# jasonyaw/CDAE

Measured on AMD Instinct MI355X. Metric: users/sec (whole node) K=200 ML-10M-shape; Recall@10 parity, higher is better.
Workload: dtype f32

## Files before the change

### cdae_amd/csrc/cdae_hip.hip

```cpp
#include <hip/hip_runtime.h>

#include <cstring>

#include <rocprim/rocprim.hpp>

#include <algorithm>
#include <atomic>
#include <condition_variable>
#include <deque>
#include <mutex>
#include <thread>
#include <chrono>
#include <cmath>
#include <cstdarg>
#include <cstdlib>
#include <cstdio>
#include <cstring>
#include <numeric>
#include <string>
#include <vector>

#include "../../include/cdae_hip.h"
#include "cdae_internal.hpp"
#include "cdae_kernels.hpp"
// ... 163 lines not shown
  double* d_rows_out = nullptr;
  int sort_bits = 1;
  struct PrepJob { int set; uint64_t s0; uint32_t nb, cidx; uint64_t E; uint64_t seed; uint32_t epoch; int lane; uint64_t prof_q; };
  bool prep_threaded = true;
  std::thread worker;
  std::mutex job_mu;
  std::condition_variable job_cv;
  std::condition_variable issued_cv;
  std::deque<PrepJob> jobs;
  bool worker_stop = false;
  uint64_t jobs_submitted = 0;
  std::atomic<uint64_t> jobs_issued{0};
  std::atomic<int> worker_failed{0};
  std::string worker_error;
  std::mutex prof_mu;
  bool encode_two_launches = false;
  bool debug_skip_prep = false;
  bool bucket_sort = false;
  uint32_t bucket_ranges = 0;
  uint32_t* d_bucket_cut = nullptr;
  bool bucket_attr_set = false;
  uint16_t* d_range_of = nullptr;
  uint32_t cell_units = 0;
  bool counting_sort = false;
  bool tile_attr_set = false;
  bool gemm3_attr_set[8] = {false, false, false, false, false, false, false, false};
  bool gemmw_attr_set[8] = {false, false, false, false, false, false, false, false};
  bool gemm_narrow = false;
  bool gemm1_tiled = false;
  bool gemm1_duo_attr_set[2] = {false, false};
  bool fused_attr_set = false;
  bool gemm2_nt = false;
  bool gemm_tn_attr_set = false;
  bool rows_separate = false;
  bool fused_rows_attr_set[2][2] = {};
  int rows_fused_kh = 2;

  float* d_base = nullptr; float* d_delta = nullptr; float* d_recv = nullptr; float* d_snap = nullptr;
  void* xchg = nullptr; void (*xchg_free)(void*) = nullptr;
  uint32_t delta_combine = CDAE_COMBINE_SUM;
  uint32_t mf = 0, mf_bias = 1;
  bool mf_seq = false;
  bool mf_auto = false;
  bool prep_force_sort = false;
  std::vector<uint32_t> user_perm, user_inv;
  uint32_t ex_per_pos = 1;
// ... 243 lines not shown
    hipLaunchKernelGGL(mf_sample_kernel, dim3((n_units + 3) / 4), dim3(256), 0, st, h->hp, h->mf == 2 ? 1u : 0u, h->d_row_ptr, h->d_col,
                       h->d_unit_ptr + bt.s0, n_units, bt.s0, bt.nb, seed, epoch, x.item, x.val, x.key16, x.seg, bucket ? 0u : 2u * I, x.dup_count,
                       x.dup_of_ex, h->d_unit_user, x.wg_state);
  } else if (shs) {
    hipLaunchKernelGGL(sample_kernel, dim3((n_units + 3) / 4), dim3(256), 0, st, h->hp, h->d_grow_ptr, h->d_gcol,
                       h->d_gunit_ptr + bt.s0, n_units, bt.s0, bt.nb, bt.cidx, seed, epoch, x.item, x.val, x.key16,
                       x.seg, h->counting_sort || bucket ? 0u : 4u * I, x.dup_count, x.dup_of_ex, h->d_gunit_user,
                       x.wg_state, (const uint32_t*)nullptr, (uint32_t)h->item0, I, (uint32_t)h->I_global,
                       (const uint16_t*)(use_cells ? h->d_range_of : nullptr), (const uint32_t*)h->d_bucket_cut, h->bucket_ranges,
                       use_cells ? x.cells : (uint32_t*)nullptr, x.cell_flag, x.cell_tag);
  } else
  hipLaunchKernelGGL(sample_kernel, dim3((n_units + 3) / 4), dim3(256), 0, st, h->hp, h->d_row_ptr, h->d_col,
                     h->d_unit_ptr + bt.s0, n_units, bt.s0, bt.nb, bt.cidx, seed, epoch, x.item, x.val, x.key16,
                     x.seg, h->counting_sort || bucket ? 0u : 4u * I, x.dup_count, x.dup_of_ex, h->d_unit_user,
                     x.wg_state, (const uint32_t*)h->d_gpos, 0u, 0u, 0u,
                     (const uint16_t*)(use_cells ? h->d_range_of : nullptr), (const uint32_t*)h->d_bucket_cut, h->bucket_ranges,
                     use_cells ? x.cells : (uint32_t*)nullptr, x.cell_flag, x.cell_tag);
  CHK(pr.end());
  CHK(pr.begin(h, F_SORT, st, prof_q));
  const dim3 seg_grid((uint32_t)((bt.E + 256 * SEG_PER_THREAD - 1) / (256 * SEG_PER_THREAD)));
  if (bt.E == 0) {
  } else if (h->mf_seq && !h->prep_force_sort) {
  } else if (bucket) {
    if (!h->bucket_attr_set) {
      HIPCHK(hipFuncSetAttribute((const void*)bucket_sort_kernel, hipFuncAttributeMaxDynamicSharedMemorySize, (int)BK_LDS_BYTES));
      h->bucket_attr_set = true;
    }
    hipLaunchKernelGGL(bucket_sort_kernel, dim3(h->bucket_ranges), dim3(BK_THREADS), BK_LDS_BYTES, st, (const uint16_t*)x.key16, (const uint64_t*)x.val,
                       (uint32_t)bt.E, (const uint32_t*)h->d_bucket_cut, x.wg_state, (const uint32_t*)(use_cells ? x.cells : nullptr), n_units,
                       (const uint32_t*)x.cell_flag, x.cell_tag, x.seg, x.seg + I, (const uint32_t*)h->d_rank_of,
                       x.seg + 2 * (size_t)I, x.seg + 3 * (size_t)I, x.sorted_val, x.bucketed, x.dup_count, h->dup_cap, x.dup_of_pos, x.dup_of_ex,
                       h->dup_stripes, h->d_fused_err);
  } else if (h->counting_sort) {
    const uint32_t n_tiles = (uint32_t)((bt.E + TILE_EX - 1) / TILE_EX);
    const size_t tile_lds = (size_t)I * sizeof(uint32_t);
    if (tile_lds + 1024 > 64 * 1024 && !h->tile_attr_set) {
      HIPCHK(hipFuncSetAttribute((const void*)tile_hist_kernel, hipFuncAttributeMaxDynamicSharedMemorySize, (int)tile_lds));
      HIPCHK(hipFuncSetAttribute((const void*)tile_scatter_kernel, hipFuncAttributeMaxDynamicSharedMemorySize, (int)tile_lds + 1024));
      h->tile_attr_set = true;
    }
    hipLaunchKernelGGL(tile_hist_kernel, dim3(n_tiles), dim3(TILE_THREADS), tile_lds / 2 + 4, st, x.item, (uint32_t)bt.E, I, x.tile_hist);
    hipLaunchKernelGGL(item_tile_scan_kernel, dim3((I + 255) / 256), dim3(256), 0, st, x.tile_hist, n_tiles, I, x.item_count, x.rank, x.block_total);
    hipLaunchKernelGGL(tile_scatter_kernel, dim3(n_tiles), dim3(TILE_THREADS), tile_lds + 128 * sizeof(uint32_t), st, x.item, x.val,
                       (uint32_t)bt.E, I, x.tile_hist, x.item_count, x.rank, x.block_total, x.prefix, x.seg, x.seg + I, x.dup_count, x.bucketed,
                       (const uint32_t*)h->d_rank_of, x.seg + 2 * (size_t)I, x.seg + 3 * (size_t)I);
    hipLaunchKernelGGL(segment_sort_kernel, dim3((I + SEGSORT_ITEMS - 1) / SEGSORT_ITEMS), dim3(SEGSORT_THREADS), 0, st, I, x.prefix, x.bucketed,
                       x.sorted_val, x.item_count, x.dup_count, h->dup_cap, x.dup_of_pos, x.dup_of_ex, h->dup_stripes);
  } else if (x.key16) {
    HIPCHK(rocprim::radix_sort_pairs(sort_tmp, h->sort_tmp_bytes, x.key16, x.sorted_key16, x.val, x.sorted_val,
                                     (size_t)bt.E, 0u, (unsigned)h->sort_bits, st));
    hipLaunchKernelGGL(segment_kernel<uint16_t>, seg_grid, dim3(256), 0, st, x.sorted_key16, x.sorted_val, (uint32_t)bt.E,
                       x.seg, x.seg + I, x.dup_count, h->dup_cap, x.dup_of_pos, x.dup_of_ex, h->dup_stripes,
                       (const uint32_t*)h->d_rank_of, x.seg + 2 * (size_t)I, x.seg + 3 * (size_t)I, shs ? I : 0xFFFFFFFFu);
  } else {
    HIPCHK(rocprim::radix_sort_pairs(sort_tmp, h->sort_tmp_bytes, x.item, x.sorted_item, x.val, x.sorted_val,
// ... 911 lines not shown
    h->g_row_ptr_src = nullptr; h->g_col_src = nullptr;
    if (grp[0] != 0) return fail("whole-row row_ptr[0] must be 0");
    h->h_grow_ptr.assign(grp, grp + U + 1);
    uint64_t gmax = 0;
    for (uint64_t s0 = 0; s0 < U; ++s0) gmax = std::max<uint64_t>(gmax, (uint64_t)(grp[std::min<uint64_t>(U, s0 + B)] - grp[s0]));
    h->Ecap = gmax * h->ex_per_pos;
    const size_t gnnz = (size_t)grp[U];
    CHK(dev_alloc(&h->d_grow_ptr, U + 1)); CHK(dev_alloc(&h->d_gcol, gnnz));
    HIPCHK(hipMemcpy(h->d_grow_ptr, grp, (U + 1) * sizeof(int64_t), hipMemcpyHostToDevice));
    HIPCHK(hipMemcpy(h->d_gcol, gcl, gnnz * sizeof(uint32_t), hipMemcpyHostToDevice));
    h->h_gunit_ptr.assign(U + 1, 0u);
    for (uint64_t u = 0; u < U; ++u)
      h->h_gunit_ptr[u + 1] = h->h_gunit_ptr[u] + (uint32_t)((grp[u + 1] - grp[u] + h->hp.unit_pos - 1) / h->hp.unit_pos);
    CHK(dev_alloc(&h->d_gunit_ptr, U + 1));
    HIPCHK(hipMemcpy(h->d_gunit_ptr, h->h_gunit_ptr.data(), (U + 1) * sizeof(uint32_t), hipMemcpyHostToDevice));
    std::vector<uint32_t> guser(h->h_gunit_ptr[U]);
    for (uint64_t u = 0; u < U; ++u)
      for (uint32_t g = h->h_gunit_ptr[u]; g < h->h_gunit_ptr[u + 1]; ++g) guser[g] = (uint32_t)u;
    CHK(dev_alloc(&h->d_gunit_user, std::max<size_t>(guser.size(), 1)));
    HIPCHK(hipMemcpy(h->d_gunit_user, guser.data(), guser.size() * sizeof(uint32_t), hipMemcpyHostToDevice));
  }
  h->seq = 0; h->pre_n = 0;
  h->counting_sort = I <= cdae::TILE_SORT_MAX_ITEMS && DEV_ENV("CDAE_SORT_TILE") != nullptr;
  h->bucket_sort = false; h->bucket_ranges = 0; h->cell_units = 0;
  {
    const uint64_t BUCKET_MAX_EXAMPLES = h->cfg.full_output ? 100000 : 600000;
    const uint64_t keys = I + (h->shard_sampled() ? 1u : 0u);
    if (keys <= 65536 && !h->counting_sort && !h->mf_seq && h->Ecap <= BUCKET_MAX_EXAMPLES && h->Ecap > 0 && !DEV_ENV("CDAE_SORT_LIBRARY")) {
      const double b_share = (double)B / (double)U;
      const double draw_items = (double)(h->shard_sampled() ? h->I_global : I);
      const double whole_nnz = h->shard_sampled() ? (double)h->h_grow_ptr[U] : (double)nnz;
      const uint32_t negs = h->mf == 2 ? 2u * h->hp.num_neg - 0u : h->hp.num_neg;
      const double neg_per_item = b_share * whole_nnz * (double)negs / draw_items;
      std::vector<double> wgt(I);
      double total = 0.0;
      for (uint64_t i = 0; i < I; ++i) { wgt[i] = b_share * (double)pop[i] + neg_per_item; total += wgt[i]; }
      const double per_range = std::max(total / 256.0, std::min(2730.0, total / 8.0));
      std::vector<uint32_t> cut{0u};
      double acc = 0.0;
      for (uint64_t i = 0; i < I; ++i) {
        acc += wgt[i];
        if (i + 1 < I && (acc >= per_range || (i + 1) - cut.back() == cdae::BK_ITEMS)) { cut.push_back((uint32_t)(i + 1)); acc = 0.0; }
      }
      cut.push_back((uint32_t)I);
      if (cut.size() - 1 <= cdae::BK_MAX_RANGES) {
        h->bucket_sort = true;
        h->bucket_ranges = (uint32_t)cut.size() - 1;
        CHK(dev_alloc(&h->d_bucket_cut, cut.size()));
        HIPCHK(hipMemcpy(h->d_bucket_cut, cut.data(), cut.size() * sizeof(uint32_t), hipMemcpyHostToDevice));
        if (!h->mf && h->bucket_ranges <= cdae::BKC_MAX_RANGES && h->Ecap < (1ull << (32 - cdae::BKC_ITEM_BITS)) && !DEV_ENV("CDAE_SORT_SCAN")) {
          std::vector<uint16_t> rof(I);
          for (uint32_t r = 0; r + 1 < cut.size(); ++r)
            for (uint32_t i = cut[r]; i < cut[r + 1]; ++i) rof[i] = (uint16_t)r;
          CHK(dev_alloc(&h->d_range_of, (size_t)I));
          HIPCHK(hipMemcpy(h->d_range_of, rof.data(), I * sizeof(uint16_t), hipMemcpyHostToDevice));
        }
      }
    }
  }
  h->h_unit_ptr.assign(U + 1, 0u);
  for (uint64_t u = 0; u < U; ++u)
    h->h_unit_ptr[u + 1] = h->h_unit_ptr[u] + (uint32_t)((row_ptr[u + 1] - row_ptr[u] + h->hp.unit_pos - 1) / h->hp.unit_pos);
  h->unit_cap = 0;
  for (uint64_t s0 = 0; s0 < U; ++s0) {
    const uint64_t s1 = std::min<uint64_t>(U, s0 + B);
    h->unit_cap = std::max(h->unit_cap, h->h_unit_ptr[s1] - h->h_unit_ptr[s0]);
  }
  {
    std::vector<uint32_t> per(U);
    for (uint64_t u = 0; u < U; ++u) per[u] = h->h_unit_ptr[u + 1] - h->h_unit_ptr[u];
    std::partial_sort(per.begin(), per.begin() + B, per.end(), std::greater<uint32_t>());
    uint64_t top = 0;
    for (uint32_t i = 0; i < B; ++i) top += per[i];
    h->unit_cap = (uint32_t)std::max<uint64_t>(h->unit_cap, top);
  }
  if (h->shard_sampled())
    for (uint64_t s0 = 0; s0 < U; ++s0)
      h->unit_cap = std::max(h->unit_cap, h->h_gunit_ptr[std::min<uint64_t>(U, s0 + B)] - h->h_gunit_ptr[s0]);
  CHK(dev_alloc(&h->d_unit_ptr, U + 1));
  HIPCHK(hipMemcpy(h->d_unit_ptr, h->h_unit_ptr.data(), (U + 1) * sizeof(uint32_t), hipMemcpyHostToDevice));
  {
    std::vector<uint32_t> unit_user(h->h_unit_ptr[U]);
    for (uint64_t u = 0; u < U; ++u)
      for (uint32_t g = h->h_unit_ptr[u]; g < h->h_unit_ptr[u + 1]; ++g) unit_user[g] = (uint32_t)u;
    CHK(dev_alloc(&h->d_unit_user, std::max<size_t>(unit_user.size(), 1)));
    HIPCHK(hipMemcpy(h->d_unit_user, unit_user.data(), unit_user.size() * sizeof(uint32_t), hipMemcpyHostToDevice));
  }
  CHK(dev_alloc(&h->d_Hpart, (size_t)h->unit_cap * h->Kp));
  CHK(dev_alloc(&h->d_uptr_tmp, (size_t)B + 1));
  {
    const uint32_t one_unit[2] = {0u, 1u};
    HIPCHK(hipMemcpy(h->d_uptr_tmp, one_unit, sizeof one_unit, hipMemcpyHostToDevice));
  }
  if ((uint64_t)B * h->Kp * sizeof(float) > 0x7FFFFFFFull)
    return fail("batch_users %u x row stride %u floats exceeds the 2 GiB the batch's Z may occupy; lower batch_users", B, h->Kp);
  if (h->Ecap > 0xFFFFFFF0ull) return fail("batch of %u users holds %llu examples (> 2^32); lower batch_users", B, (unsigned long long)h->Ecap);
  for (auto& b : h->ex) {
    CHK(dev_alloc(&b.item, h->Ecap)); CHK(dev_alloc(&b.val, h->Ecap));
    CHK(dev_alloc(&b.sorted_item, h->Ecap)); CHK(dev_alloc(&b.sorted_val, h->Ecap));
    CHK(dev_alloc(&b.seg, 4 * (size_t)I));
    CHK(dev_alloc(&b.dup_of_pos, h->Ecap)); CHK(dev_alloc(&b.dup_of_ex, h->Ecap)); CHK(dev_alloc(&b.dup_count, cdae::DUP_STRIPES));
// ... 1454 lines not shown
```

### cdae_amd/csrc/cdae_kernels.hpp

```cpp
#pragma once
#include <type_traits>

#include <hip/hip_runtime.h>
#include <stdint.h>

#include "../../include/cdae_rng.h"
#include "cdae_exchange_algebra.h"

namespace cdae {

constexpr int WAVE = 64;
constexpr uint32_t SLOT_MASK = 0x0FFFFFFFu;
constexpr uint32_t DUP_PREV_BIT = 1u << 28;
constexpr uint32_t DUP_NEXT_BIT = 1u << 29;
constexpr uint32_t DUP_NONE = 0xFFFFFFFFu;
constexpr uint32_t DUP_STRIPES = 64;
constexpr uint32_t TARGET_BIT = 1u << 30;
constexpr uint32_t INPUT_BIT = 1u << 31;

constexpr uint32_t LATE_MAX = 64;
struct DecodeLate {
  float* Ghot;
  uint32_t* hotdup;
  uint32_t late_rows;
// ... 1423 lines not shown
                     const uint32_t* __restrict__ dup_of_ex, const float* __restrict__ dup_corr,
                     const uint32_t* __restrict__ unit_user,
                     const uint32_t* __restrict__ late_bits = nullptr ,
                     uint32_t late_words = 0) {
  __shared__ uint32_t gl_row[4][GATHER_CAP];
  __shared__ float gl_g[4][GATHER_CAP];
  __shared__ uint32_t lbits[LATE_BITS_WORDS];
  stage_late_bits(lbits, late_bits, late_words);
  const uint32_t part = blockIdx.x & 7u;
  const uint32_t unit = (blockIdx.x >> 3) * (blockDim.x / WAVE) + threadIdx.x / WAVE;
  if (unit >= n_units) return;
  const GatherArgs ga{row_ptr, uptr, n_units, u0, nb, ex_item, G, D0, HGpart, explicit_examples, dup_of_ex, dup_corr, unit_user,
                      late_bits, late_words, nullptr};
  hidden_gather_role<NI, false>(hp, ga, part, unit, gl_row[threadIdx.x / WAVE], gl_g[threadIdx.x / WAVE], late_bits ? lbits : nullptr);
}

struct FusedGeom {
  uint32_t hot_wgs;
  uint32_t decode_wgs;
  const uint32_t* cold_map;
};
constexpr uint32_t FUSED_LDS_WORDS = 4u * 2u * GATHER_CAP + LATE_BITS_WORDS;
static_assert(4u * ROWS16_LDS_WORDS <= FUSED_LDS_WORDS, "row roles' LDS");
static_assert(3u * (FUSED_LDS_WORDS + 8u) * 4u + 90376u <= 160u * 1024u, "three workgroups of this launch + one of bucket_sort_kernel per CU");
#ifndef CDAE_FUSED_WAVES_PER_SIMD
#define CDAE_FUSED_WAVES_PER_SIMD 3
#endif
template <int NV, int NT, int LOSS, bool ADAGRAD>
__global__ void __launch_bounds__(256, CDAE_FUSED_WAVES_PER_SIMD)
decode_gather_kernel(HyperParams hp, uint32_t hot_rows, FusedGeom geo, DecodeLate late, GatherArgs ga, CDAE_DECODE_PARAMS) {
  constexpr int CH = NT == 0 ? NV : NV + 1;
  constexpr int NI = CH <= 1 ? 1 : (CH <= 2 ? 2 : 4);
  __shared__ uint32_t fused_lds[FUSED_LDS_WORDS + 8u];
  const uint32_t wg = blockIdx.x;
  const uint32_t wid = __builtin_amdgcn_readfirstlane(threadIdx.x / WAVE);
  if (wg < geo.hot_wgs) {
    const uint32_t row = wg * 4u + wid;
    if (row < hot_rows && !CDAE_SKIP_ROLE(hp, 4u)) {
      const unsigned long long t0 = trace_begin(hp);
      __builtin_amdgcn_s_setprio(CDAE_HOT_PRIO);
      decode_row64<NI, LOSS, ADAGRAD, false, true>(hp, row, reinterpret_cast<float*>(fused_lds + wid * ROWS16_LDS_WORDS), ROW64_PARK_WORDS, late,
                                                   CDAE_DECODE_PASS);
      __builtin_amdgcn_s_setprio(0);
      trace_end(hp, 3, row, t0, hp.trace ? hw_place() : 0u);
    }
  } else if (wg < geo.decode_wgs) {
    if (CDAE_SKIP_ROLE(hp, 8u)) return;
// ... 748 lines not shown
```

### cdae_amd/csrc/cdae_sort_kernels.hpp

```cpp
#pragma once
#include <hip/hip_runtime.h>
#include <stdint.h>

#include "cdae_kernels.hpp"

namespace cdae {

#ifndef CDAE_SEGSORT_THREADS
#define CDAE_SEGSORT_THREADS 256
#endif
constexpr uint32_t SEGSORT_THREADS = CDAE_SEGSORT_THREADS;
#ifndef CDAE_SEGSORT_ITEMS
#define CDAE_SEGSORT_ITEMS 8
#endif
constexpr uint32_t SEGSORT_ITEMS = CDAE_SEGSORT_ITEMS;
#ifndef CDAE_SEGSORT_WINDOW
#define CDAE_SEGSORT_WINDOW 3072
#endif
constexpr uint32_t SEGSORT_WINDOW = CDAE_SEGSORT_WINDOW;

constexpr uint32_t TILE_SORT_MAX_ITEMS = 32768;
#ifndef CDAE_TILE_EX
#define CDAE_TILE_EX 4096
#endif
// ... 179 lines not shown
      for (uint32_t q = threadIdx.x; q < n; q += blockDim.x) {
        const uint64_t v = sorted_val[p0 + q];
        if (!((uint32_t)v & DUP_PREV_BIT)) continue;
        const uint32_t idx = off < stripe_cap ? stripe0 + off : DUP_NONE;
        ++off;
        dup_of_pos[p0 + q] = idx;
        dup_of_ex[(uint32_t)(v >> 32)] = idx;
      }
    }
    __syncthreads();
    k0 = k1;
  }
}

constexpr uint32_t BK_THREADS = 512;
constexpr uint32_t BK_WINDOW = 4096;
constexpr uint32_t BK_ITEMS = 2048;
constexpr uint32_t BK_WAVE_LIST = BK_WINDOW / (BK_THREADS / 64);
constexpr uint32_t BK_SPIN_CAP = 1u << 21;
constexpr uint32_t BK_MAX_RANGES = 1024;
constexpr uint32_t BK_CELL_UNITS_MAX = 16384;
constexpr size_t BK_LDS_BYTES = (size_t)BK_WINDOW * 8 * 2 + (size_t)BK_WINDOW * 2 + (size_t)(BK_ITEMS + 1) * 4 * 2 + 64 * 4;
static_assert(BK_ITEMS <= 4 * BK_THREADS && BK_ITEMS <= (1u << BKC_ITEM_BITS), "bk_block_scan takes 4 counters per thread; a cell entry holds the item in BKC_ITEM_BITS bits");

__device__ __forceinline__ void bk_block_scan(uint32_t* v, uint32_t n, uint32_t* wave_tot) {
  const uint32_t t = threadIdx.x, lane = t % WAVE, wid = t / WAVE;
  uint32_t c[4], sum = 0;
#pragma unroll
  for (uint32_t j = 0; j < 4; ++j) { c[j] = 4u * t + j < n ? v[4u * t + j] : 0u; sum += c[j]; }
  uint32_t incl = sum;
#pragma unroll
  for (int off = 1; off < WAVE; off <<= 1) {
    const uint32_t o = __shfl_up(incl, off, WAVE);
    if ((int)lane >= off) incl += o;
  }
  if (lane == WAVE - 1) wave_tot[wid] = incl;
  __syncthreads();
  uint32_t before = 0;
  for (uint32_t w = 0; w < wid; ++w) before += wave_tot[w];
  uint32_t run = before + incl - sum;
#pragma unroll
  for (uint32_t j = 0; j < 4; ++j) { if (4u * t + j < n) v[4u * t + j] = run; run += c[j]; }
  if (t == BK_THREADS - 1) v[n] = run;
  __syncthreads();
}

constexpr uint32_t BK_UNROLL = 4;
template <typename F>
__device__ __forceinline__ void bk_scan_keys(const uint16_t* __restrict__ keys, uint32_t n_ex, F&& f) {
  const uint32_t n8 = n_ex & ~7u;
  constexpr uint32_t ROUND = BK_THREADS * 8u * BK_UNROLL;
  uint4 q[BK_UNROLL], nx[BK_UNROLL];
  auto request = [&](uint4 (&dst)[BK_UNROLL], uint32_t r0) {
#pragma unroll
    for (uint32_t u = 0; u < BK_UNROLL; ++u) {
      const uint32_t e0 = r0 + (u * BK_THREADS + threadIdx.x) * 8u;
      dst[u] = e0 < n8 ? *reinterpret_cast<const uint4*>(keys + e0) : make_uint4(0xFFFFFFFFu, 0xFFFFFFFFu, 0xFFFFFFFFu, 0xFFFFFFFFu);
    }
  };
  request(q, 0u);
  for (uint32_t r0 = 0; r0 < n8; r0 += ROUND) {
    const bool more = r0 + ROUND < n8;
    if (more) request(nx, r0 + ROUND);
#pragma unroll
    for (uint32_t u = 0; u < BK_UNROLL; ++u) {
      const uint32_t e0 = r0 + (u * BK_THREADS + threadIdx.x) * 8u;
      if (r0 + u * BK_THREADS * 8u >= n8) break;
      const bool valid = e0 < n8;
      const uint32_t w[4] = {q[u].x, q[u].y, q[u].z, q[u].w};
#pragma unroll
      for (uint32_t j = 0; j < 4; ++j) { f(e0 + 2u * j, w[j] & 0xFFFFu, valid); f(e0 + 2u * j + 1u, w[j] >> 16, valid); }
    }
    if (more) {
#pragma unroll
      for (uint32_t u = 0; u < BK_UNROLL; ++u) q[u] = nx[u];
    }
  }
  if (n_ex != n8 && threadIdx.x < WAVE) {
    const bool valid = threadIdx.x < n_ex - n8;
    f(n8 + threadIdx.x, valid ? (uint32_t)keys[n8 + threadIdx.x] : 0u, valid);
  }
}

__global__ void __launch_bounds__(BK_THREADS)
bucket_sort_kernel(const uint16_t* __restrict__ keys, const uint64_t* __restrict__ ex_val, uint32_t n_ex,
                   const uint32_t* __restrict__ range_cut , uint32_t* __restrict__ wg_state ,
                   const uint32_t* __restrict__ cells , uint32_t cell_units,
                   const uint32_t* __restrict__ cell_flag , uint32_t cell_tag,
                   uint32_t* __restrict__ seg_begin, uint32_t* __restrict__ seg_end, const uint32_t* __restrict__ rank_of,
                   uint32_t* __restrict__ segr_begin, uint32_t* __restrict__ segr_end, uint64_t* __restrict__ sorted_val,
                   uint64_t* __restrict__ scratch_val ,
                   uint32_t* __restrict__ dup_count, uint32_t dup_cap, uint32_t* __restrict__ dup_of_pos,
                   uint32_t* __restrict__ dup_of_ex , uint32_t stripes,
                   uint32_t* __restrict__ err ) {
#ifdef CDAE_PREP_SETPRIO
  __builtin_amdgcn_s_setprio(CDAE_PREP_SETPRIO);
#endif
  extern __shared__ __attribute__((aligned(16))) unsigned char bk_lds[];
  uint64_t* raw = reinterpret_cast<uint64_t*>(bk_lds);
  uint64_t* srt = raw + BK_WINDOW;
  uint32_t* off = reinterpret_cast<uint32_t*>(srt + BK_WINDOW);
  uint32_t* cur = off + BK_ITEMS + 1;
  uint32_t* misc = cur + BK_ITEMS + 1;
  uint16_t* raw_item = reinterpret_cast<uint16_t*>(misc + 64);
  const uint32_t t = threadIdx.x, w = blockIdx.x, lane = t % WAVE;
  const uint32_t lo = range_cut[w], n_it = range_cut[w + 1] - lo;
  for (uint32_t i = t; i <= n_it; i += BK_THREADS) off[i] = 0u;
  if (t == 0) { misc[16] = 0u; misc[17] = 0u; misc[19] = 0u; }
  __syncthreads();

  bool listed = false;
  bool scanned = false;
  if (cells && cell_units <= BK_CELL_UNITS_MAX && *cell_flag != cell_tag) {
    uint16_t* wcnt = reinterpret_cast<uint16_t*>(raw);
    uint32_t* lst = reinterpret_cast<uint32_t*>(srt);
    uint16_t* tk = reinterpret_cast<uint16_t*>(lst + BK_WINDOW);
    const uint32_t* mine = cells + (size_t)w * cell_units * BKC_SLOTS;
    const uint32_t per = (cell_units + BK_THREADS - 1) / BK_THREADS, u0 = min(cell_units, t * per), u1 = min(cell_units, u0 + per);
    uint32_t sum = 0;
    for (uint32_t u = u0; u < u1; ++u) { const uint32_t c = mine[(size_t)u * BKC_SLOTS]; wcnt[u] = (uint16_t)c; sum += c; }
    uint32_t incl = sum;
#pragma unroll
    for (int o = 1; o < WAVE; o <<= 1) {
      const uint32_t v = __shfl_up(incl, o, WAVE);
      if ((int)lane >= o) incl += v;
    }
    if (lane == WAVE - 1) misc[t / WAVE] = incl;
    __syncthreads();
    uint32_t pos = incl - sum, total = 0;
    for (uint32_t v = 0; v < BK_THREADS / WAVE; ++v) { if (v < t / WAVE) pos += misc[v]; total += misc[v]; }
    __syncthreads();
    if (total <= BK_WINDOW) {
      for (uint32_t u = u0; u < u1; ++u) {
        const uint32_t c = wcnt[u];
        for (uint32_t j = 0; j < c; ++j) lst[pos + j] = mine[(size_t)u * BKC_SLOTS + 1u + j];
        pos += c;
      }
      __syncthreads();
      for (uint32_t i = t; i < total; i += BK_THREADS) tk[i] = (uint16_t)atomicAdd(&off[lst[i] & BKC_ITEM_MASK], 1u);
      __syncthreads();
      bk_block_scan(off, n_it, misc);
      for (uint32_t i = t; i < total; i += BK_THREADS) {
        const uint32_t ent = lst[i], d = ent & BKC_ITEM_MASK, p = off[d] + tk[i];
        raw[p] = ex_val[ent >> BKC_ITEM_BITS];
        raw_item[p] = (uint16_t)d;
      }
      listed = true; scanned = true;
    } else {
      for (uint32_t i = t; i <= n_it; i += BK_THREADS) off[i] = 0u;
      __syncthreads();
    }
  }

  uint64_t* const wave_list = srt + (t / WAVE) * BK_WAVE_LIST;
  uint32_t wave_n = 0;
  if (!scanned) {
    bk_scan_keys(keys, n_ex, [&](uint32_t e, uint32_t k, bool valid) {
      const uint32_t d = k - lo;
      const bool mine = valid && d < n_it;
      const uint64_t m = __ballot(mine);
      if (m == 0ull) return;
      if (mine) {
        const uint32_t ticket = atomicAdd(&off[d], 1u);
        const uint32_t slot = wave_n + __builtin_amdgcn_mbcnt_hi((uint32_t)(m >> 32), __builtin_amdgcn_mbcnt_lo((uint32_t)m, 0u));
        if (slot < BK_WAVE_LIST) wave_list[slot] = ((uint64_t)e << 32) | (uint64_t)(d << 16) | (uint64_t)(ticket & 0xFFFFu);
      }
      wave_n += (uint32_t)__popcll(m);
    });
    if (wave_n > BK_WAVE_LIST && lane == 0) misc[19] = 1u;
    __syncthreads();
    bk_block_scan(off, n_it, misc);
  }

  if (t == 0) __hip_atomic_store(&wg_state[w], off[n_it] + 1u, __ATOMIC_RELEASE, __HIP_MEMORY_SCOPE_AGENT);
  for (uint32_t r = t; r < w; r += BK_THREADS) {
    uint32_t v, spin = 0;
    while ((v = __hip_atomic_load(&wg_state[r], __ATOMIC_ACQUIRE, __HIP_MEMORY_SCOPE_AGENT)) == 0u) {
      if (++spin > BK_SPIN_CAP) { v = 1u; __hip_atomic_store(err, 2u, __ATOMIC_RELAXED, __HIP_MEMORY_SCOPE_SYSTEM); break; }
      __builtin_amdgcn_s_sleep(1);
    }
    atomicAdd(&misc[16], v - 1u);
  }
  __syncthreads();
  const uint32_t base = misc[16];
  for (uint32_t i = t; i < n_it; i += BK_THREADS) {
    const uint32_t c = off[i + 1] - off[i], b = c ? base + off[i] : 0u, e = c ? base + off[i + 1] : 0u;
    seg_begin[lo + i] = b; seg_end[lo + i] = e;
    if (rank_of) { const uint32_t r = rank_of[lo + i]; segr_begin[r] = b; segr_end[r] = e; }
  }
  const bool wave_listed = !listed && misc[19] == 0u && off[n_it] <= BK_WINDOW;

  uint32_t ia = 0;
  while (ia < n_it) {
    uint32_t ib = ia + 1;
    {
      uint32_t l = ia + 1, h = n_it;
      while (l < h) { const uint32_t mid = (l + h + 1) >> 1; if (off[mid] - off[ia] <= BK_WINDOW) l = mid; else h = mid - 1; }
      ib = l;
    }
    const uint32_t g0 = off[ia], n = off[ib] - g0;
    const bool in_lds = n <= BK_WINDOW;
    if (n == 0) { ia = ib; continue; }
    if (listed) {
    } else if (wave_listed) {
      for (uint32_t i = lane; i < wave_n; i += WAVE) {
        const uint64_t rec = wave_list[i];
        const uint32_t d = (uint32_t)(rec >> 16) & 0xFFFFu, p = off[d] + ((uint32_t)rec & 0xFFFFu);
        raw[p] = ex_val[(uint32_t)(rec >> 32)];
        raw_item[p] = (uint16_t)d;
      }
    } else {
      for (uint32_t i = ia + t; i < ib; i += BK_THREADS) cur[i] = off[i] - g0;
      __syncthreads();
      bk_scan_keys(keys, n_ex, [&](uint32_t e, uint32_t k, bool valid) {
        const uint32_t d = k - lo;
        if (valid && d - ia < ib - ia) {
          const uint32_t p = atomicAdd(&cur[d], 1u);
          const uint64_t v = ex_val[e];
          if (in_lds) { raw[p] = v; raw_item[p] = (uint16_t)d; } else scratch_val[base + g0 + p] = v;
        }
      });
    }
    __threadfence_block();
    __syncthreads();
    for (uint32_t q = t; q < n; q += BK_THREADS) {
      if (in_lds) {
        const uint32_t d = raw_item[q], a = off[d] - g0, b = off[d + 1] - g0;
        const uint64_t v = raw[q];
        uint32_t r[8] = {0, 0, 0, 0, 0, 0, 0, 0};
        uint32_t j = a;
        for (; j + 8 <= b; j += 8) {
#pragma unroll
          for (int u = 0; u < 8; ++u) r[u] += raw[j + u] < v ? 1u : 0u;
        }
        for (; j < b; ++j) r[0] += raw[j] < v ? 1u : 0u;
        srt[a + ((r[0] + r[1]) + (r[2] + r[3])) + ((r[4] + r[5]) + (r[6] + r[7]))] = v;
      } else {
        const uint64_t v = scratch_val[base + g0 + q];
        uint32_t rank = 0;
        for (uint32_t j = 0; j < n; ++j) rank += scratch_val[base + g0 + j] < v ? 1u : 0u;
        sorted_val[base + g0 + rank] = v;
      }
    }
    __threadfence_block();
    __syncthreads();
    uint32_t my_dups = 0;
    for (uint32_t q = t; q < n; q += BK_THREADS) {
      uint32_t a = 0, b = n;
      if (in_lds) {
        uint32_t l = ia, h = ib - 1;
        while (l < h) { const uint32_t mid = (l + h + 1) >> 1; if (off[mid] - g0 <= q) l = mid; else h = mid - 1; }
        a = off[l] - g0; b = off[l + 1] - g0;
      }
      const uint64_t v = in_lds ? srt[q] : sorted_val[base + g0 + q];
      const uint32_t slot = (uint32_t)v & SLOT_MASK;
      uint32_t flags = 0;
      if (q > a && ((uint32_t)(in_lds ? srt[q - 1] : sorted_val[base + g0 + q - 1]) & SLOT_MASK) == slot) flags |= DUP_PREV_BIT;
      if (q + 1 < b && ((uint32_t)(in_lds ? srt[q + 1] : sorted_val[base + g0 + q + 1]) & SLOT_MASK) == slot) flags |= DUP_NEXT_BIT;
      if (in_lds || flags) sorted_val[base + g0 + q] = v | flags;
      if (flags & DUP_PREV_BIT) ++my_dups;
    }
    uint32_t o = my_dups ? atomicAdd(&misc[17], my_dups) : 0u;
    __syncthreads();
    if (t == 0) { misc[18] = misc[17] ? atomicAdd(dup_count + w % stripes, misc[17]) : 0u; misc[17] = 0u; }
    __syncthreads();
    if (my_dups) {
      o += misc[18];
      const uint32_t stripe_cap = dup_cap / stripes, stripe0 = (w % stripes) * stripe_cap;
      for (uint32_t q = t; q < n; q += BK_THREADS) {
        const uint64_t v = sorted_val[base + g0 + q];
        if (!((uint32_t)v & DUP_PREV_BIT)) continue;
        const uint32_t idx = o < stripe_cap ? stripe0 + o : DUP_NONE;
        ++o;
        dup_of_pos[base + g0 + q] = idx;
        dup_of_ex[(uint32_t)(v >> 32)] = idx;
      }
    }
    __syncthreads();
    ia = ib;
  }
}

}
```

Baseline: 2.924 million.

## Add a smaller-LDS cells form of the bucket sort kernel

Templates bucket_sort_kernel on a CELLS flag. The cells form uses a 2048-entry window, 1024 items per range and 256 threads, which brings LDS to about 45 KB so two of its workgroups can sit beside three fused-launch workgroups on a CU. It also spreads cell-list gathering across threads by binary search over unit prefixes, and the host picks range cuts with a lower fill target when the cells path fits. The aim is more concurrency between the prep sort and the fused compute kernel, at the cost of more ranges and a fallback to a global-memory rank path when a range overflows the smaller window.

New measurement: 2.658 million. -9.1%, worse.

```diff
diff --git a/cdae_amd/csrc/cdae_hip.hip b/cdae_amd/csrc/cdae_hip.hip
--- a/cdae_amd/csrc/cdae_hip.hip
+++ b/cdae_amd/csrc/cdae_hip.hip
@@ -209,6 +209,7 @@
   bool bucket_attr_set = false;
   uint16_t* d_range_of = nullptr;
   uint32_t cell_units = 0;
+  bool bucket_cells_form = false;
   bool counting_sort = false;
   bool tile_attr_set = false;
   bool gemm3_attr_set[8] = {false, false, false, false, false, false, false, false};
@@ -498,15 +499,22 @@
   if (bt.E == 0) {
   } else if (h->mf_seq && !h->prep_force_sort) {
   } else if (bucket) {
-    if (!h->bucket_attr_set) {
-      HIPCHK(hipFuncSetAttribute((const void*)bucket_sort_kernel, hipFuncAttributeMaxDynamicSharedMemorySize, (int)BK_LDS_BYTES));
+    if (!h->bucket_cells_form && !h->bucket_attr_set) {
+      HIPCHK(hipFuncSetAttribute((const void*)bucket_sort_kernel<false>, hipFuncAttributeMaxDynamicSharedMemorySize, (int)BK_LDS_BYTES));
       h->bucket_attr_set = true;
     }
-    hipLaunchKernelGGL(bucket_sort_kernel, dim3(h->bucket_ranges), dim3(BK_THREADS), BK_LDS_BYTES, st, (const uint16_t*)x.key16, (const uint64_t*)x.val,
-                       (uint32_t)bt.E, (const uint32_t*)h->d_bucket_cut, x.wg_state, (const uint32_t*)(use_cells ? x.cells : nullptr), n_units,
-                       (const uint32_t*)x.cell_flag, x.cell_tag, x.seg, x.seg + I, (const uint32_t*)h->d_rank_of,
-                       x.seg + 2 * (size_t)I, x.seg + 3 * (size_t)I, x.sorted_val, x.bucketed, x.dup_count, h->dup_cap, x.dup_of_pos, x.dup_of_ex,
-                       h->dup_stripes, h->d_fused_err);
+    if (h->bucket_cells_form)
+      hipLaunchKernelGGL(bucket_sort_kernel<true>, dim3(h->bucket_ranges), dim3(BK_CELLS_THREADS), BK_CELLS_LDS_BYTES, st, (const uint16_t*)x.key16, (const uint64_t*)x.val,
+                         (uint32_t)bt.E, (const uint32_t*)h->d_bucket_cut, x.wg_state, (const uint32_t*)(use_cells ? x.cells : nullptr), n_units,
+                         (const uint32_t*)x.cell_flag, x.cell_tag, x.seg, x.seg + I, (const uint32_t*)h->d_rank_of,
+                         x.seg + 2 * (size_t)I, x.seg + 3 * (size_t)I, x.sorted_val, x.bucketed, x.dup_count, h->dup_cap, x.dup_of_pos, x.dup_of_ex,
+                         h->dup_stripes, h->d_fused_err);
+    else
+      hipLaunchKernelGGL(bucket_sort_kernel<false>, dim3(h->bucket_ranges), dim3(BK_THREADS), BK_LDS_BYTES, st, (const uint16_t*)x.key16, (const uint64_t*)x.val,
+                         (uint32_t)bt.E, (const uint32_t*)h->d_bucket_cut, x.wg_state, (const uint32_t*)(use_cells ? x.cells : nullptr), n_units,
+                         (const uint32_t*)x.cell_flag, x.cell_tag, x.seg, x.seg + I, (const uint32_t*)h->d_rank_of,
+                         x.seg + 2 * (size_t)I, x.seg + 3 * (size_t)I, x.sorted_val, x.bucketed, x.dup_count, h->dup_cap, x.dup_of_pos, x.dup_of_ex,
+                         h->dup_stripes, h->d_fused_err);
   } else if (h->counting_sort) {
     const uint32_t n_tiles = (uint32_t)((bt.E + TILE_EX - 1) / TILE_EX);
     const size_t tile_lds = (size_t)I * sizeof(uint32_t);
@@ -1464,7 +1472,26 @@
   }
   h->seq = 0; h->pre_n = 0;
   h->counting_sort = I <= cdae::TILE_SORT_MAX_ITEMS && DEV_ENV("CDAE_SORT_TILE") != nullptr;
-  h->bucket_sort = false; h->bucket_ranges = 0; h->cell_units = 0;
+  h->h_unit_ptr.assign(U + 1, 0u);
+  for (uint64_t u = 0; u < U; ++u)
+    h->h_unit_ptr[u + 1] = h->h_unit_ptr[u] + (uint32_t)((row_ptr[u + 1] - row_ptr[u] + h->hp.unit_pos - 1) / h->hp.unit_pos);
+  h->unit_cap = 0;
+  for (uint64_t s0 = 0; s0 < U; ++s0) {
+    const uint64_t s1 = std::min<uint64_t>(U, s0 + B);
+    h->unit_cap = std::max(h->unit_cap, h->h_unit_ptr[s1] - h->h_unit_ptr[s0]);
+  }
+  {
+    std::vector<uint32_t> per(U);
+    for (uint64_t u = 0; u < U; ++u) per[u] = h->h_unit_ptr[u + 1] - h->h_unit_ptr[u];
+    std::partial_sort(per.begin(), per.begin() + B, per.end(), std::greater<uint32_t>());
+    uint64_t top = 0;
+    for (uint32_t i = 0; i < B; ++i) top += per[i];
+    h->unit_cap = (uint32_t)std::max<uint64_t>(h->unit_cap, top);
+  }
+  if (h->shard_sampled())
+    for (uint64_t s0 = 0; s0 < U; ++s0)
+      h->unit_cap = std::max(h->unit_cap, h->h_gunit_ptr[std::min<uint64_t>(U, s0 + B)] - h->h_gunit_ptr[s0]);
+  h->bucket_sort = false; h->bucket_ranges = 0; h->cell_units = 0; h->bucket_cells_form = false;
   {
     const uint64_t BUCKET_MAX_EXAMPLES = h->cfg.full_output ? 100000 : 600000;
     const uint64_t keys = I + (h->shard_sampled() ? 1u : 0u);
@@ -1477,20 +1504,35 @@
       std::vector<double> wgt(I);
       double total = 0.0;
       for (uint64_t i = 0; i < I; ++i) { wgt[i] = b_share * (double)pop[i] + neg_per_item; total += wgt[i]; }
-      const double per_range = std::max(total / 256.0, std::min(2730.0, total / 8.0));
-      std::vector<uint32_t> cut{0u};
-      double acc = 0.0;
-      for (uint64_t i = 0; i < I; ++i) {
-        acc += wgt[i];
-        if (i + 1 < I && (acc >= per_range || (i + 1) - cut.back() == cdae::BK_ITEMS)) { cut.push_back((uint32_t)(i + 1)); acc = 0.0; }
+      std::vector<uint32_t> cut;
+      auto cut_for = [&](double fill, uint32_t most_items) {
+        const double per_range = std::max(total / 256.0, std::min(fill, total / 8.0));
+        cut.assign(1, 0u);
+        double acc = 0.0;
+        for (uint64_t i = 0; i < I; ++i) {
+          acc += wgt[i];
+          if (i + 1 < I && (acc >= per_range || (i + 1) - cut.back() == most_items)) { cut.push_back((uint32_t)(i + 1)); acc = 0.0; }
+        }
+        cut.push_back((uint32_t)I);
+      };
+      const bool cells_ok = !h->mf && h->Ecap < (1ull << (32 - cdae::BKC_ITEM_BITS)) && !DEV_ENV("CDAE_SORT_SCAN");
+      auto cells_fit = [&]() {
+        return cut.size() - 1 <= cdae::BKC_MAX_RANGES && h->unit_cap <= cdae::BK_CELL_UNITS_MAX &&
+               (cut.size() - 1) * (size_t)h->unit_cap * cdae::BKC_SLOTS * sizeof(uint32_t) <= (256ull << 20);
+      };
+      h->bucket_cells_form = cells_ok && h->unit_cap <= cdae::BkCfg<true>::CELL_UNITS_MAX &&
+                             total <= (double)cdae::BKC_MAX_RANGES * cdae::BK_CELLS_FILL && !DEV_ENV("CDAE_SORT_WIDE");
+      if (h->bucket_cells_form) {
+        cut_for((double)cdae::BK_CELLS_FILL, cdae::BK_CELLS_ITEMS);
+        h->bucket_cells_form = cells_fit();
       }
-      cut.push_back((uint32_t)I);
+      if (!h->bucket_cells_form) cut_for(2730.0, cdae::BK_ITEMS);
       if (cut.size() - 1 <= cdae::BK_MAX_RANGES) {
         h->bucket_sort = true;
         h->bucket_ranges = (uint32_t)cut.size() - 1;
         CHK(dev_alloc(&h->d_bucket_cut, cut.size()));
         HIPCHK(hipMemcpy(h->d_bucket_cut, cut.data(), cut.size() * sizeof(uint32_t), hipMemcpyHostToDevice));
-        if (!h->mf && h->bucket_ranges <= cdae::BKC_MAX_RANGES && h->Ecap < (1ull << (32 - cdae::BKC_ITEM_BITS)) && !DEV_ENV("CDAE_SORT_SCAN")) {
+        if (cells_ok && h->bucket_ranges <= cdae::BKC_MAX_RANGES) {
           std::vector<uint16_t> rof(I);
           for (uint32_t r = 0; r + 1 < cut.size(); ++r)
             for (uint32_t i = cut[r]; i < cut[r + 1]; ++i) rof[i] = (uint16_t)r;
@@ -1500,25 +1542,6 @@
       }
     }
   }
-  h->h_unit_ptr.assign(U + 1, 0u);
-  for (uint64_t u = 0; u < U; ++u)
-    h->h_unit_ptr[u + 1] = h->h_unit_ptr[u] + (uint32_t)((row_ptr[u + 1] - row_ptr[u] + h->hp.unit_pos - 1) / h->hp.unit_pos);
-  h->unit_cap = 0;
-  for (uint64_t s0 = 0; s0 < U; ++s0) {
-    const uint64_t s1 = std::min<uint64_t>(U, s0 + B);
-    h->unit_cap = std::max(h->unit_cap, h->h_unit_ptr[s1] - h->h_unit_ptr[s0]);
-  }
-  {
-    std::vector<uint32_t> per(U);
-    for (uint64_t u = 0; u < U; ++u) per[u] = h->h_unit_ptr[u + 1] - h->h_unit_ptr[u];
-    std::partial_sort(per.begin(), per.begin() + B, per.end(), std::greater<uint32_t>());
-    uint64_t top = 0;
-    for (uint32_t i = 0; i < B; ++i) top += per[i];
-    h->unit_cap = (uint32_t)std::max<uint64_t>(h->unit_cap, top);
-  }
-  if (h->shard_sampled())
-    for (uint64_t s0 = 0; s0 < U; ++s0)
-      h->unit_cap = std::max(h->unit_cap, h->h_gunit_ptr[std::min<uint64_t>(U, s0 + B)] - h->h_gunit_ptr[s0]);
   CHK(dev_alloc(&h->d_unit_ptr, U + 1));
   HIPCHK(hipMemcpy(h->d_unit_ptr, h->h_unit_ptr.data(), (U + 1) * sizeof(uint32_t), hipMemcpyHostToDevice));
   {
diff --git a/cdae_amd/csrc/cdae_kernels.hpp b/cdae_amd/csrc/cdae_kernels.hpp
--- a/cdae_amd/csrc/cdae_kernels.hpp
+++ b/cdae_amd/csrc/cdae_kernels.hpp
@@ -1469,7 +1469,8 @@
 };
 constexpr uint32_t FUSED_LDS_WORDS = 4u * 2u * GATHER_CAP + LATE_BITS_WORDS;
 static_assert(4u * ROWS16_LDS_WORDS <= FUSED_LDS_WORDS, "row roles' LDS");
-static_assert(3u * (FUSED_LDS_WORDS + 8u) * 4u + 90376u <= 160u * 1024u, "three workgroups of this launch + one of bucket_sort_kernel per CU");
+static_assert(3u * (FUSED_LDS_WORDS + 8u) * 4u + 2u * 45320u <= 160u * 1024u && 2u * 45320u >= 90376u,
+              "three workgroups of this launch + two of bucket_sort_kernel's cells form (or one of its wide form) per CU");
 #ifndef CDAE_FUSED_WAVES_PER_SIMD
 #define CDAE_FUSED_WAVES_PER_SIMD 3
 #endif
diff --git a/cdae_amd/csrc/cdae_sort_kernels.hpp b/cdae_amd/csrc/cdae_sort_kernels.hpp
--- a/cdae_amd/csrc/cdae_sort_kernels.hpp
+++ b/cdae_amd/csrc/cdae_sort_kernels.hpp
@@ -225,7 +225,23 @@
 constexpr uint32_t BK_CELL_UNITS_MAX = 16384;
 constexpr size_t BK_LDS_BYTES = (size_t)BK_WINDOW * 8 * 2 + (size_t)BK_WINDOW * 2 + (size_t)(BK_ITEMS + 1) * 4 * 2 + 64 * 4;
 static_assert(BK_ITEMS <= 4 * BK_THREADS && BK_ITEMS <= (1u << BKC_ITEM_BITS), "bk_block_scan takes 4 counters per thread; a cell entry holds the item in BKC_ITEM_BITS bits");
-
+constexpr uint32_t BK_CELLS_THREADS = 256;
+constexpr uint32_t BK_CELLS_WINDOW = 2048;
+constexpr uint32_t BK_CELLS_ITEMS = 1024;
+constexpr uint32_t BK_CELLS_FILL = BK_CELLS_WINDOW * 2 / 3;
+template <bool CELLS> struct BkCfg {
+  static constexpr uint32_t THREADS = CELLS ? BK_CELLS_THREADS : BK_THREADS;
+  static constexpr uint32_t WINDOW = CELLS ? BK_CELLS_WINDOW : BK_WINDOW;
+  static constexpr uint32_t ITEMS = CELLS ? BK_CELLS_ITEMS : BK_ITEMS;
+  static constexpr uint32_t CELL_UNITS_MAX = 4 * WINDOW;
+  static constexpr size_t LDS_BYTES = (size_t)WINDOW * 8 * 2 + (size_t)WINDOW * 2 + (size_t)(ITEMS + 1) * 4 * 2 + 64 * 4;
+};
+constexpr size_t BK_CELLS_LDS_BYTES = BkCfg<true>::LDS_BYTES;
+static_assert(BkCfg<false>::LDS_BYTES == BK_LDS_BYTES && BkCfg<false>::CELL_UNITS_MAX == BK_CELL_UNITS_MAX, "the wide form is what it was");
+static_assert(BK_CELLS_LDS_BYTES <= 48 * 1024 && BK_CELLS_LDS_BYTES == 45320, "the cells form: at most 48 KB of LDS per workgroup (cdae_kernels.hpp sums it with the fused launch's)");
+static_assert(BK_CELLS_ITEMS <= 4 * BK_CELLS_THREADS && BK_CELLS_ITEMS <= (1u << BKC_ITEM_BITS) && BK_CELLS_WINDOW < 65536, "4 counters per thread; item bits of a cell entry; 16-bit unit prefixes");
+
+template <uint32_t THREADS>
 __device__ __forceinline__ void bk_block_scan(uint32_t* v, uint32_t n, uint32_t* wave_tot) {
   const uint32_t t = threadIdx.x, lane = t % WAVE, wid = t / WAVE;
   uint32_t c[4], sum = 0;
@@ -244,20 +260,20 @@
   uint32_t run = before + incl - sum;
 #pragma unroll
   for (uint32_t j = 0; j < 4; ++j) { if (4u * t + j < n) v[4u * t + j] = run; run += c[j]; }
-  if (t == BK_THREADS - 1) v[n] = run;
+  if (t == THREADS - 1) v[n] = run;
   __syncthreads();
 }
 
 constexpr uint32_t BK_UNROLL = 4;
-template <typename F>
+template <uint32_t THREADS, typename F>
 __device__ __forceinline__ void bk_scan_keys(const uint16_t* __restrict__ keys, uint32_t n_ex, F&& f) {
   const uint32_t n8 = n_ex & ~7u;
-  constexpr uint32_t ROUND = BK_THREADS * 8u * BK_UNROLL;
+  constexpr uint32_t ROUND = THREADS * 8u * BK_UNROLL;
   uint4 q[BK_UNROLL], nx[BK_UNROLL];
   auto request = [&](uint4 (&dst)[BK_UNROLL], uint32_t r0) {
 #pragma unroll
     for (uint32_t u = 0; u < BK_UNROLL; ++u) {
-      const uint32_t e0 = r0 + (u * BK_THREADS + threadIdx.x) * 8u;
+      const uint32_t e0 = r0 + (u * THREADS + threadIdx.x) * 8u;
       dst[u] = e0 < n8 ? *reinterpret_cast<const uint4*>(keys + e0) : make_uint4(0xFFFFFFFFu, 0xFFFFFFFFu, 0xFFFFFFFFu, 0xFFFFFFFFu);
     }
   };
@@ -267,8 +283,8 @@
     if (more) request(nx, r0 + ROUND);
 #pragma unroll
     for (uint32_t u = 0; u < BK_UNROLL; ++u) {
-      const uint32_t e0 = r0 + (u * BK_THREADS + threadIdx.x) * 8u;
-      if (r0 + u * BK_THREADS * 8u >= n8) break;
+      const uint32_t e0 = r0 + (u * THREADS + threadIdx.x) * 8u;
+      if (r0 + u * THREADS * 8u >= n8) break;
       const bool valid = e0 < n8;
       const uint32_t w[4] = {q[u].x, q[u].y, q[u].z, q[u].w};
 #pragma unroll
@@ -285,7 +301,8 @@
   }
 }
 
-__global__ void __launch_bounds__(BK_THREADS)
+template <bool CELLS>
+__global__ void __launch_bounds__(BkCfg<CELLS>::THREADS)
 bucket_sort_kernel(const uint16_t* __restrict__ keys, const uint64_t* __restrict__ ex_val, uint32_t n_ex,
                    const uint32_t* __restrict__ range_cut , uint32_t* __restrict__ wg_state ,
                    const uint32_t* __restrict__ cells , uint32_t cell_units,
@@ -299,27 +316,30 @@
 #ifdef CDAE_PREP_SETPRIO
   __builtin_amdgcn_s_setprio(CDAE_PREP_SETPRIO);
 #endif
+  constexpr uint32_t THREADS = BkCfg<CELLS>::THREADS, WINDOW = BkCfg<CELLS>::WINDOW, ITEMS = BkCfg<CELLS>::ITEMS;
+  constexpr uint32_t CELL_UNITS_MAX = BkCfg<CELLS>::CELL_UNITS_MAX;
+  constexpr uint32_t WAVE_LIST = WINDOW / (THREADS / WAVE);
   extern __shared__ __attribute__((aligned(16))) unsigned char bk_lds[];
   uint64_t* raw = reinterpret_cast<uint64_t*>(bk_lds);
-  uint64_t* srt = raw + BK_WINDOW;
-  uint32_t* off = reinterpret_cast<uint32_t*>(srt + BK_WINDOW);
-  uint32_t* cur = off + BK_ITEMS + 1;
-  uint32_t* misc = cur + BK_ITEMS + 1;
+  uint64_t* srt = raw + WINDOW;
+  uint32_t* off = reinterpret_cast<uint32_t*>(srt + WINDOW);
+  uint32_t* cur = off + ITEMS + 1;
+  uint32_t* misc = cur + ITEMS + 1;
   uint16_t* raw_item = reinterpret_cast<uint16_t*>(misc + 64);
   const uint32_t t = threadIdx.x, w = blockIdx.x, lane = t % WAVE;
   const uint32_t lo = range_cut[w], n_it = range_cut[w + 1] - lo;
-  for (uint32_t i = t; i <= n_it; i += BK_THREADS) off[i] = 0u;
+  for (uint32_t i = t; i <= n_it; i += THREADS) off[i] = 0u;
   if (t == 0) { misc[16] = 0u; misc[17] = 0u; misc[19] = 0u; }
   __syncthreads();
 
   bool listed = false;
   bool scanned = false;
-  if (cells && cell_units <= BK_CELL_UNITS_MAX && *cell_flag != cell_tag) {
+  if (cells && cell_units <= CELL_UNITS_MAX && *cell_flag != cell_tag) {
     uint16_t* wcnt = reinterpret_cast<uint16_t*>(raw);
     uint32_t* lst = reinterpret_cast<uint32_t*>(srt);
-    uint16_t* tk = reinterpret_cast<uint16_t*>(lst + BK_WINDOW);
+    uint16_t* tk = reinterpret_cast<uint16_t*>(lst + WINDOW);
     const uint32_t* mine = cells + (size_t)w * cell_units * BKC_SLOTS;
-    const uint32_t per = (cell_units + BK_THREADS - 1) / BK_THREADS, u0 = min(cell_units, t * per), u1 = min(cell_units, u0 + per);
+    const uint32_t per = (cell_units + THREADS - 1) / THREADS, u0 = min(cell_units, t * per), u1 = min(cell_units, u0 + per);
     uint32_t sum = 0;
     for (uint32_t u = u0; u < u1; ++u) { const uint32_t c = mine[(size_t)u * BKC_SLOTS]; wcnt[u] = (uint16_t)c; sum += c; }
     uint32_t incl = sum;
@@ -331,52 +351,68 @@
     if (lane == WAVE - 1) misc[t / WAVE] = incl;
     __syncthreads();
     uint32_t pos = incl - sum, total = 0;
-    for (uint32_t v = 0; v < BK_THREADS / WAVE; ++v) { if (v < t / WAVE) pos += misc[v]; total += misc[v]; }
-    __syncthreads();
-    if (total <= BK_WINDOW) {
-      for (uint32_t u = u0; u < u1; ++u) {
-        const uint32_t c = wcnt[u];
-        for (uint32_t j = 0; j < c; ++j) lst[pos + j] = mine[(size_t)u * BKC_SLOTS + 1u + j];
-        pos += c;
+    for (uint32_t v = 0; v < THREADS / WAVE; ++v) { if (v < t / WAVE) pos += misc[v]; total += misc[v]; }
+    __syncthreads();
+    if (total <= WINDOW) {
+      if constexpr (CELLS) {
+        for (uint32_t u = u0; u < u1; ++u) { const uint32_t c = wcnt[u]; wcnt[u] = (uint16_t)pos; pos += c; }
+        __syncthreads();
+        for (uint32_t i = t; i < total; i += THREADS) {
+          uint32_t l = 0, h = cell_units - 1u;
+          while (l < h) { const uint32_t mid = (l + h + 1) >> 1; if (wcnt[mid] <= i) l = mid; else h = mid - 1; }
+          const uint32_t ent = mine[(size_t)l * BKC_SLOTS + 1u + (i - wcnt[l])];
+          lst[i] = ent;
+          tk[i] = (uint16_t)atomicAdd(&off[ent & BKC_ITEM_MASK], 1u);
+        }
+      } else {
+        for (uint32_t u = u0; u < u1; ++u) {
+          const uint32_t c = wcnt[u];
+          for (uint32_t j = 0; j < c; ++j) lst[pos + j] = mine[(size_t)u * BKC_SLOTS + 1u + j];
+          pos += c;
+        }
+        __syncthreads();
+        for (uint32_t i = t; i < total; i += THREADS) tk[i] = (uint16_t)atomicAdd(&off[lst[i] & BKC_ITEM_MASK], 1u);
       }
       __syncthreads();
-      for (uint32_t i = t; i < total; i += BK_THREADS) tk[i] = (uint16_t)atomicAdd(&off[lst[i] & BKC_ITEM_MASK], 1u);
-      __syncthreads();
-      bk_block_scan(off, n_it, misc);
-      for (uint32_t i = t; i < total; i += BK_THREADS) {
+      bk_block_scan<THREADS>(off, n_it, misc);
+      for (uint32_t i = t; i < total; i += THREADS) {
         const uint32_t ent = lst[i], d = ent & BKC_ITEM_MASK, p = off[d] + tk[i];
         raw[p] = ex_val[ent >> BKC_ITEM_BITS];
         raw_item[p] = (uint16_t)d;
       }
       listed = true; scanned = true;
     } else {
-      for (uint32_t i = t; i <= n_it; i += BK_THREADS) off[i] = 0u;
+      for (uint32_t i = t; i <= n_it; i += THREADS) off[i] = 0u;
       __syncthreads();
     }
   }
 
-  uint64_t* const wave_list = srt + (t / WAVE) * BK_WAVE_LIST;
+  uint64_t* const wave_list = srt + (t / WAVE) * WAVE_LIST;
   uint32_t wave_n = 0;
   if (!scanned) {
-    bk_scan_keys(keys, n_ex, [&](uint32_t e, uint32_t k, bool valid) {
+    bk_scan_keys<THREADS>(keys, n_ex, [&](uint32_t e, uint32_t k, bool valid) {
       const uint32_t d = k - lo;
       const bool mine = valid && d < n_it;
       const uint64_t m = __ballot(mine);
       if (m == 0ull) return;
       if (mine) {
         const uint32_t ticket = atomicAdd(&off[d], 1u);
-        const uint32_t slot = wave_n + __builtin_amdgcn_mbcnt_hi((uint32_t)(m >> 32), __builtin_amdgcn_mbcnt_lo((uint32_t)m, 0u));
-        if (slot < BK_WAVE_LIST) wave_list[slot] = ((uint64_t)e << 32) | (uint64_t)(d << 16) | (uint64_t)(ticket & 0xFFFFu);
+        if constexpr (CELLS) {
+          (void)ticket; (void)e;
+        } else {
+          const uint32_t slot = wave_n + __builtin_amdgcn_mbcnt_hi((uint32_t)(m >> 32), __builtin_amdgcn_mbcnt_lo((uint32_t)m, 0u));
+          if (slot < WAVE_LIST) wave_list[slot] = ((uint64_t)e << 32) | (uint64_t)(d << 16) | (uint64_t)(ticket & 0xFFFFu);
+        }
       }
       wave_n += (uint32_t)__popcll(m);
     });
-    if (wave_n > BK_WAVE_LIST && lane == 0) misc[19] = 1u;
-    __syncthreads();
-    bk_block_scan(off, n_it, misc);
+    if ((CELLS || wave_n > WAVE_LIST) && lane == 0) misc[19] = 1u;
+    __syncthreads();
+    bk_block_scan<THREADS>(off, n_it, misc);
   }
 
   if (t == 0) __hip_atomic_store(&wg_state[w], off[n_it] + 1u, __ATOMIC_RELEASE, __HIP_MEMORY_SCOPE_AGENT);
-  for (uint32_t r = t; r < w; r += BK_THREADS) {
+  for (uint32_t r = t; r < w; r += THREADS) {
     uint32_t v, spin = 0;
     while ((v = __hip_atomic_load(&wg_state[r], __ATOMIC_ACQUIRE, __HIP_MEMORY_SCOPE_AGENT)) == 0u) {
       if (++spin > BK_SPIN_CAP) { v = 1u; __hip_atomic_store(err, 2u, __ATOMIC_RELAXED, __HIP_MEMORY_SCOPE_SYSTEM); break; }
@@ -386,23 +422,23 @@
   }
   __syncthreads();
   const uint32_t base = misc[16];
-  for (uint32_t i = t; i < n_it; i += BK_THREADS) {
+  for (uint32_t i = t; i < n_it; i += THREADS) {
     const uint32_t c = off[i + 1] - off[i], b = c ? base + off[i] : 0u, e = c ? base + off[i + 1] : 0u;
     seg_begin[lo + i] = b; seg_end[lo + i] = e;
     if (rank_of) { const uint32_t r = rank_of[lo + i]; segr_begin[r] = b; segr_end[r] = e; }
   }
-  const bool wave_listed = !listed && misc[19] == 0u && off[n_it] <= BK_WINDOW;
+  const bool wave_listed = !listed && misc[19] == 0u && off[n_it] <= WINDOW;
 
   uint32_t ia = 0;
   while (ia < n_it) {
     uint32_t ib = ia + 1;
     {
       uint32_t l = ia + 1, h = n_it;
-      while (l < h) { const uint32_t mid = (l + h + 1) >> 1; if (off[mid] - off[ia] <= BK_WINDOW) l = mid; else h = mid - 1; }
+      while (l < h) { const uint32_t mid = (l + h + 1) >> 1; if (off[mid] - off[ia] <= WINDOW) l = mid; else h = mid - 1; }
       ib = l;
     }
     const uint32_t g0 = off[ia], n = off[ib] - g0;
-    const bool in_lds = n <= BK_WINDOW;
+    const bool in_lds = n <= WINDOW;
     if (n == 0) { ia = ib; continue; }
     if (listed) {
     } else if (wave_listed) {
@@ -413,9 +449,9 @@
         raw_item[p] = (uint16_t)d;
       }
     } else {
-      for (uint32_t i = ia + t; i < ib; i += BK_THREADS) cur[i] = off[i] - g0;
+      for (uint32_t i = ia + t; i < ib; i += THREADS) cur[i] = off[i] - g0;
       __syncthreads();
-      bk_scan_keys(keys, n_ex, [&](uint32_t e, uint32_t k, bool valid) {
+      bk_scan_keys<THREADS>(keys, n_ex, [&](uint32_t e, uint32_t k, bool valid) {
         const uint32_t d = k - lo;
         if (valid && d - ia < ib - ia) {
           const uint32_t p = atomicAdd(&cur[d], 1u);
@@ -426,7 +462,7 @@
     }
     __threadfence_block();
     __syncthreads();
-    for (uint32_t q = t; q < n; q += BK_THREADS) {
+    for (uint32_t q = t; q < n; q += THREADS) {
       if (in_lds) {
         const uint32_t d = raw_item[q], a = off[d] - g0, b = off[d + 1] - g0;
         const uint64_t v = raw[q];
@@ -448,7 +484,7 @@
     __threadfence_block();
     __syncthreads();
     uint32_t my_dups = 0;
-    for (uint32_t q = t; q < n; q += BK_THREADS) {
+    for (uint32_t q = t; q < n; q += THREADS) {
       uint32_t a = 0, b = n;
       if (in_lds) {
         uint32_t l = ia, h = ib - 1;
@@ -470,7 +506,7 @@
     if (my_dups) {
       o += misc[18];
       const uint32_t stripe_cap = dup_cap / stripes, stripe0 = (w % stripes) * stripe_cap;
-      for (uint32_t q = t; q < n; q += BK_THREADS) {
+      for (uint32_t q = t; q < n; q += THREADS) {
         const uint64_t v = sorted_val[base + g0 + q];
         if (!((uint32_t)v & DUP_PREV_BIT)) continue;
         const uint32_t idx = o < stripe_cap ? stripe0 + o : DUP_NONE;
```
